# davidbau/rewriting

Measured on AMD Instinct MI355X. Metric: images/sec StyleGANv2-1024 fwd, higher is better.
Workload: dtype f32 (conv operands split into exact f16 pairs from 32x32 up, f32 accumulate); 1 GPU; stylegan2-1024 generator forward (FFHQ-1024 architecture); batch_per_gpu=64, mconv=seq, weights=synthetic seed 0, parallelism=seeds partitioned per rank, no collective, matrix_mode=split, direct_sums=auto

## Files before the change

include/rewriting_hip.h:

```cpp
#ifndef REWRITING_HIP_H
#define REWRITING_HIP_H

#include <stdint.h>

#ifdef __cplusplus
extern "C" {
#endif

typedef void* rw_stream_t;

#define RW_ERR_BAD_ARGUMENT 10001
#define RW_ERR_UNSUPPORTED  10002

int rw_abi_version(void);
const char* rw_error_string(int code);


int rw_fused_bias_act_f32(const float* x, const float* b, const float* ref, float* y,
                          int64_t n, int64_t step_b, int64_t size_b,
                          int act, int grad, float alpha, float scale, rw_stream_t stream);
int rw_fused_bias_act_f16(const uint16_t* x, const uint16_t* b, const uint16_t* ref, uint16_t* y,
                          int64_t n, int64_t step_b, int64_t size_b,
                          int act, int grad, float alpha, float scale, rw_stream_t stream);
int rw_fused_bias_act_f64(const double* x, const double* b, const double* ref, double* y,
// ... 120 lines not shown
int rw_conv_weight_wino4h_absmax_f32(const float* w, int out_ch, int in_ch, float* bound, rw_stream_t stream);
int rw_conv_transpose_blur_weight_wino4h_absmax_f32(const float* w, const float* k4, int out_ch, int in_ch, float* bound,
                                                    rw_stream_t stream);
int rw_conv_transpose_weight_winoh_absmax_f32(const float* w, int out_ch, int in_ch, float* bound, rw_stream_t stream);
int rw_dconv_weight_absmax_f32(const float* w, int out_ch, int in_ch, float* bound, rw_stream_t stream);
int rw_dconv_transpose_blur_weight_absmax_f32(const float* w, const float* k4, int out_ch, int in_ch, float* bound,
                                              rw_stream_t stream);
long long rw_packed_conv_weight_wino4h_elems(int out_ch, int in_ch);
int rw_pack_conv_weight_wino4h_f32(const float* w, float* uf, int out_ch, int in_ch, float u_scale, rw_stream_t stream);
int rw_conv3x3_wino4h_f32(const float* x, const float* uf, float* y, int batch, int in_ch, int out_ch, int h,
                          int w, float w_scale, const rw_conv_epilogue* ep, float u_inv, const float* x_amax,
                          float* y_amax, rw_stream_t stream);
int rw_conv3x3_wino4h_to_rgb_f32(const float* x, const float* uf, int batch, int in_ch, int out_ch, int h, int w,
                                 float w_scale, const rw_conv_epilogue* ep, const rw_rgb_epilogue* rgb, float u_inv,
                                 const float* x_amax, rw_stream_t stream);
long long rw_packed_conv_transpose_blur_wino4h_elems(int out_ch, int in_ch);
int rw_pack_conv_transpose_blur_weight_wino4h_f32(const float* w, const float* k4, float* uf, int out_ch, int in_ch,
                                                  float u_scale, rw_stream_t stream);
int rw_conv_transpose3x3s2_blur_wino4h_f32(const float* x, const float* uf, float* y, int batch, int in_ch,
                                           int out_ch, int h, int w, float w_scale, const rw_conv_epilogue* ep,
                                           const float* post_scale, float u_inv, const float* x_amax,
                                           float* y_amax, rw_stream_t stream);

int rw_dconv3x3_supported(int out_ch, int in_ch, int h, int w);
long long rw_packed_dconv_weight_elems(int out_ch, int in_ch);
int rw_pack_dconv_weight_f32(const float* w, float* wp, int out_ch, int in_ch, float u_scale, rw_stream_t stream);
int rw_dconv3x3_f32(const float* x, const float* wp, float* y, int batch, int in_ch, int out_ch, int h, int w,
                    float w_scale, const rw_conv_epilogue* ep, float u_inv, const float* x_amax, float* y_amax,
                    rw_stream_t stream);
int rw_dconv3x3_rgb_partials(int out_ch);
int rw_dconv3x3_rgb_partial_f32(const float* x, const float* wp, float* y, int batch, int in_ch, int out_ch, int h, int w,
                                float w_scale, const rw_conv_epilogue* ep, const rw_rgb_epilogue* rgb, float u_inv,
                                const float* x_amax, float* y_amax, rw_stream_t stream);
int rw_rgb_combine_f32(const float* partials, int n_part, const float* bias, const float* skip, float* y, int batch,
                       int64_t hw, rw_stream_t stream);
int rw_dconv3x3_to_rgb_supported(int out_ch, int in_ch, int h, int w);
int rw_dconv3x3_to_rgb_f32(const float* x, const float* wp, int batch, int in_ch, int out_ch, int h, int w,
                           float w_scale, const rw_conv_epilogue* ep, const rw_rgb_epilogue* rgb, float u_inv,
                           const float* x_amax, rw_stream_t stream);
int rw_dconv_transpose_blur_supported(int out_ch, int in_ch, int h, int w);
long long rw_packed_dconv_transpose_blur_weight_elems(int out_ch, int in_ch);
int rw_pack_dconv_transpose_blur_weight_f32(const float* w, const float* k4, float* wp, int out_ch, int in_ch,
                                            float u_scale, rw_stream_t stream);
int rw_dconv_transpose3x3s2_blur_f32(const float* x, const float* wp, float* y, int batch, int in_ch, int out_ch, int h,
                                     int w, float w_scale, const rw_conv_epilogue* ep, const float* post_scale,
                                     float u_inv, const float* x_amax, float* y_amax, rw_stream_t stream);

int rw_tconv_blur_supported(int out_ch, int in_ch, int h, int w);
int rw_tconv_blur_f32(const float* x, const float* wp, const float* k4, float* y, int batch, int in_ch, int out_ch, int h,
                      int w, float w_scale, const rw_conv_epilogue* ep, const float* post_scale, float u_inv,
// ... 154 lines not shown
```

rewriting_amd/_lib.py:

```python
import ctypes
import os
from ctypes import (POINTER, Structure, c_char_p, c_double, c_float, c_int, c_int32, c_int64, c_uint,
                    c_void_p)

_HERE = os.path.dirname(os.path.abspath(__file__))
LIB_PATH = os.environ.get('RW_HIP_LIB') or os.path.join(_HERE, 'librewriting_hip.so')

ABI_VERSION = 11


class ConvEpilogue(Structure):
    _fields_ = [('style', c_void_p), ('demod', c_void_p), ('noise', c_void_p),
                ('noise_w', c_void_p), ('bias', c_void_p), ('act', c_int)]


class RgbEpilogue(Structure):
    _fields_ = [('weight', c_void_p), ('style', c_void_p), ('bias', c_void_p), ('skip', c_void_p),
                ('out', c_void_p), ('scale', c_float)]


class SolveProblem(Structure):
    _fields_ = [
        ('out_ch', c_int), ('in_ch', c_int), ('h', c_int), ('w', c_int), ('rank', c_int),
        ('key', c_void_p), ('style', c_void_p), ('val', c_void_p), ('bias', c_void_p),
# ... 112 lines not shown
    'rw_pack_conv_transpose_blur_weight_wino4h_f32': (c_int, [c_void_p, c_void_p, c_void_p, c_int, c_int, c_float,
                                                              c_void_p]),
    'rw_conv_transpose3x3s2_blur_wino4h_f32': (c_int, [c_void_p, c_void_p, c_void_p, c_int, c_int, c_int, c_int,
                                                       c_int, c_float, POINTER(ConvEpilogue), c_void_p, c_float,
                                                       c_void_p, c_void_p, c_void_p]),
    'rw_dconv3x3_supported': (c_int, [c_int, c_int, c_int, c_int]),
    'rw_packed_dconv_weight_elems': (ctypes.c_longlong, [c_int, c_int]),
    'rw_pack_dconv_weight_f32': (c_int, [c_void_p, c_void_p, c_int, c_int, c_float, c_void_p]),
    'rw_dconv3x3_f32': (c_int, [c_void_p, c_void_p, c_void_p, c_int, c_int, c_int, c_int, c_int, c_float,
                                POINTER(ConvEpilogue), c_float, c_void_p, c_void_p, c_void_p]),
    'rw_dconv3x3_rgb_partials': (c_int, [c_int]),
    'rw_dconv3x3_rgb_partial_f32': (c_int, [c_void_p, c_void_p, c_void_p, c_int, c_int, c_int, c_int, c_int, c_float,
                                            POINTER(ConvEpilogue), POINTER(RgbEpilogue), c_float, c_void_p, c_void_p,
                                            c_void_p]),
    'rw_rgb_combine_f32': (c_int, [c_void_p, c_int, c_void_p, c_void_p, c_void_p, c_int, c_int64, c_void_p]),
    'rw_dconv3x3_to_rgb_supported': (c_int, [c_int, c_int, c_int, c_int]),
    'rw_dconv3x3_to_rgb_f32': (c_int, [c_void_p, c_void_p, c_int, c_int, c_int, c_int, c_int, c_float,
                                       POINTER(ConvEpilogue), POINTER(RgbEpilogue), c_float, c_void_p, c_void_p]),
    'rw_dconv_transpose_blur_supported': (c_int, [c_int, c_int, c_int, c_int]),
    'rw_packed_dconv_transpose_blur_weight_elems': (ctypes.c_longlong, [c_int, c_int]),
    'rw_pack_dconv_transpose_blur_weight_f32': (c_int, [c_void_p, c_void_p, c_void_p, c_int, c_int, c_float, c_void_p]),
    'rw_dconv_transpose3x3s2_blur_f32': (c_int, [c_void_p, c_void_p, c_void_p, c_int, c_int, c_int, c_int, c_int,
                                                 c_float, POINTER(ConvEpilogue), c_void_p, c_float, c_void_p, c_void_p,
                                                 c_void_p]),
    'rw_tconv_blur_supported': (c_int, [c_int, c_int, c_int, c_int]),
    'rw_tconv_blur_f32': (c_int, [c_void_p, c_void_p, c_void_p, c_void_p, c_int, c_int, c_int, c_int, c_int, c_float,
                                  POINTER(ConvEpilogue), c_void_p, c_float, c_void_p, c_void_p, c_void_p]),
    'rw_conv_transpose_blur_wino4_supported': (c_int, [c_int, c_int, c_int, c_int]),
    'rw_packed_conv_transpose_blur_wino4_elems': (ctypes.c_longlong, [c_int, c_int]),
    'rw_pack_conv_transpose_blur_weight_wino4_f32': (c_int, [c_void_p, c_void_p, c_void_p, c_int, c_int, c_void_p]),
# ... 79 lines not shown
```

rewriting_amd/csrc/rw_common.h:

```cpp
#pragma once
#include <hip/hip_runtime.h>
#include <stdint.h>
#include <stdlib.h>
#include "../../include/rewriting_hip.h"

#define RW_WAVE 64

#define RW_CHECK_ARG(cond) do { if (!(cond)) return RW_ERR_BAD_ARGUMENT; } while (0)
#define RW_LAUNCH_RESULT() ((int)hipGetLastError())

static inline hipStream_t rw_s(rw_stream_t s) { return (hipStream_t)s; }

static inline int64_t rw_cdiv(int64_t a, int64_t b) { return (a + b - 1) / b; }

static inline int rw_cu_count(void) {
  static int cached[64];
  int dev = 0;
  if (hipGetDevice(&dev) != hipSuccess || dev < 0 || dev >= 64) return 256;
  if (cached[dev] == 0) {
    int n = 0;
    cached[dev] = (hipDeviceGetAttribute(&n, hipDeviceAttributeMultiprocessorCount, dev) == hipSuccess && n > 0) ? n : 256;
  }
  return cached[dev];
}
// ... 197 lines not shown
__host__ __device__ __forceinline__ int rw_exp_above(float x) {
  const int e = (int)((__builtin_bit_cast(unsigned, x) >> 23) & 0xff) - 126;
  return e < -100 ? -100 : (e > 100 ? 100 : e);
}
template <int HEAD>
__host__ __device__ __forceinline__ void rw_split_scales(float am, float u_inv, float& in_scale, float& out_scale) {
  const int e = rw_exp_above(am);
  in_scale = __builtin_bit_cast(float, (unsigned)(127 + HEAD - e) << 23);
  out_scale = __builtin_bit_cast(float, (unsigned)(127 + e - HEAD) << 23) * u_inv;
}
static inline float rw_weight_scale_of(float u_absmax) {
  const int eu = u_absmax == 0.f ? 15 : rw_exp_above(u_absmax);
  return __builtin_bit_cast(float, (unsigned)(127 + 15 - eu) << 23);
}

static inline bool rw_epilogue_ok(const rw_conv_epilogue* ep) {
  return !ep || ((!ep->noise || ep->noise_w) && (!ep->act || ep->bias));
}
static inline bool rw_rgb_ok(const rw_rgb_epilogue* rgb) { return rgb && rgb->weight && rgb->style && rgb->out; }

template <class P> static inline void rw_fill_epilogue(P& p, const rw_conv_epilogue* ep) {
  p.style = ep ? ep->style : nullptr; p.demod = ep ? ep->demod : nullptr; p.noise = ep ? ep->noise : nullptr;
  p.noise_w = ep ? ep->noise_w : nullptr; p.bias = ep ? ep->bias : nullptr; p.act = ep ? ep->act : 0;
}
template <class P> static inline void rw_fill_rgb(P& p, const rw_rgb_epilogue* rgb) {
  p.rgb_weight = rgb ? rgb->weight : nullptr; p.rgb_style = rgb ? rgb->style : nullptr;
  p.rgb_bias = rgb ? rgb->bias : nullptr; p.rgb_skip = rgb ? rgb->skip : nullptr; p.rgb_out = rgb ? rgb->out : nullptr;
  p.rgb_scale = rgb ? rgb->scale : 0.f;
}

// ... 19 lines not shown
```

rewriting_amd/csrc/rw_ops.hip:

```cpp
#include "rw_common.h"
#ifndef OPS_NTS
#define OPS_NTS 0
#endif
#include <stdlib.h>
#include <stdint.h>

extern "C" int rw_abi_version(void) { return 11; }

extern "C" const char* rw_error_string(int code) {
  if (code == 0) return "success";
  if (code == RW_ERR_BAD_ARGUMENT) return "rewriting_hip: bad argument";
  if (code == RW_ERR_UNSUPPORTED) return "rewriting_hip: unsupported configuration";
  return hipGetErrorString((hipError_t)code);
}

template <typename T> struct RwAcc { typedef T type; };
template <> struct RwAcc<_Float16> { typedef float type; };

template <typename A>
__device__ __forceinline__ A rw_bias_act_one(A x, A ref, int code, A alpha, A scale) {
  A y;
  switch (code) {
    default:
    case 10: y = x; break;
// ... 1041 lines not shown
    }
    reinterpret_cast<float4*>(y)[q] = a;
  }
}

extern "C" int rw_rgb_combine_f32(const float* partials, int n_part, const float* bias, const float* skip, float* y,
                                  int batch, int64_t hw, rw_stream_t stream) {
  RW_CHECK_ARG(partials && y && n_part > 0 && batch > 0 && hw > 0);
  if (hw % 4) return RW_ERR_UNSUPPORTED;
  const int64_t n4 = (int64_t)batch * 3 * hw / 4;
  hipLaunchKernelGGL(rgb_combine_kernel, dim3(rw_stream_grid(n4, 256)), dim3(256), 0, rw_s(stream), partials, n_part, bias,
                     skip, y, n4, hw / 4, n4);
  return RW_LAUNCH_RESULT();
}

__global__ void __launch_bounds__(256) to_rgb_scalar_kernel(const float* __restrict__ x, const float* __restrict__ w,
                                                            const float* __restrict__ style,
                                                            const float* __restrict__ bias,
                                                            const float* __restrict__ skip, float* __restrict__ y,
                                                            int in_ch, int64_t hw, float w_scale) {
  extern __shared__ float wm[];
  const int b = blockIdx.y;
  for (int t = threadIdx.x; t < 3 * in_ch; t += 256) wm[t] = w_scale * w[t] * style[(int64_t)b * in_ch + t % in_ch];
  __syncthreads();
  const float* xb = x + (int64_t)b * in_ch * hw;
  for (int64_t q = (int64_t)blockIdx.x * 256 + threadIdx.x; q < hw; q += (int64_t)gridDim.x * 256) {
    float a[3] = {0.f, 0.f, 0.f};
    for (int i = 0; i < in_ch; ++i) {
      const float v = xb[(int64_t)i * hw + q];
      a[0] += wm[i] * v; a[1] += wm[in_ch + i] * v; a[2] += wm[2 * in_ch + i] * v;
// ... 31 lines not shown
```

rewriting_amd/csrc/rw_wino4.hip:

```cpp
#include "rw_common.h"

#ifndef W4_ABL
#define W4_ABL 0
#endif
#ifndef W4_SETPRIO
#define W4_SETPRIO 0
#endif

__host__ __device__ constexpr int w4_nat(int pos) { return pos < 18 ? pos : (pos < 26 ? pos + 10 : pos - 8); }

struct Wino4Problem {
  const float* x; const float* uf; float* y;
  const float* style; const float* demod; const float* noise; const float* noise_w; const float* bias;
  int batch, in_ch, out_ch, h, w;
  int groups_x, groups_y, gpw;
  float w_scale;
  int act;
  const float* rgb_weight; const float* rgb_style; const float* rgb_bias; const float* rgb_skip; float* rgb_out;
  float rgb_scale;
  const float* post;
  const float* x_amax; float* y_amax;
  float u_inv;
};

#define W4_PC 66
#define W4_RS 72

__device__ __forceinline__ void w4_bt(float& d0, float& d1, float& d2, float& d3, float& d4, float& d5) {
  const float t0 = 4.f * d0 - 5.f * d2 + d4;
  const float p = d4 - 4.f * d2, q = d3 - 4.f * d1;
  const float r = d4 - d2, s = 2.f * (d3 - d1);
  const float t5 = 4.f * d1 - 5.f * d3 + d5;
  d0 = t0; d1 = p + q; d2 = p - q; d3 = r + s; d4 = r - s; d5 = t5;
}

__device__ __forceinline__ void w4_bt2(rw_f32x2& d0, rw_f32x2& d1, rw_f32x2& d2, rw_f32x2& d3, rw_f32x2& d4,
                                       rw_f32x2& d5) {
// ... 822 lines not shown
    asm volatile("" ::: "memory");
    if (!mine) {
#pragma unroll
      for (int cc = 0; cc < 3; ++cc) *reinterpret_cast<rw_f32x4*>(&Ns[wave * NSZ + cc * 128 + slot]) = sum[cc];
    }
    __builtin_amdgcn_s_waitcnt(0xC07F);
    __builtin_amdgcn_s_barrier();
    asm volatile("" ::: "memory");
    if (mine) {
      const int64_t pix = (int64_t)(oy + lk) * p.w + ox;
#pragma unroll
      for (int cc = 0; cc < 3; ++cc) {
        const rw_f32x4 other = *reinterpret_cast<const rw_f32x4*>(&Ns[(wave ^ WGN) * NSZ + cc * 128 + slot]);
        const int64_t off = ((int64_t)ib * 3 + cc) * hw + pix;
        rw_f32x4 o4 = sum[cc] + other + (p.rgb_bias ? p.rgb_bias[cc] : 0.f);
        if (p.rgb_skip) o4 += *reinterpret_cast<const rw_f32x4*>(p.rgb_skip + off);
        *reinterpret_cast<rw_f32x4*>(p.rgb_out + off) = o4;
      }
    }
  };

  auto group_epilogue = [&](int g, int xs) __attribute__((always_inline)) {
    if (UP) { up_epilogue(g, xs); return; }
    if (RGB) { rgb_epilogue(g, xs); return; }
    const int oy = y0 + 4 * wn, ox = (gx0 + g) * 64 + 4 * lt;
    const float gain = p.act ? 1.4142135623730951f : 1.f, slope = p.act ? 0.2f : 1.f;
    rw_f32x4 nz[4];
#pragma unroll
    for (int r = 0; r < 4; ++r)
      nz[r] = p.noise ? *reinterpret_cast<const rw_f32x4*>(&Ns[wave * NSZ + 64 * r + 4 * lt]) * (noise_w * gain)
                      : rw_f32x4{0.f, 0.f, 0.f, 0.f};
// ... 451 lines not shown
}

extern "C" int rw_conv_transpose3x3s2_blur_wino4h_f32(const float* x, const float* uf, float* y, int batch, int in_ch,
                                                      int out_ch, int h, int w, float w_scale,
                                                      const rw_conv_epilogue* ep, const float* post_scale, float u_inv,
                                                      const float* x_amax, float* y_amax, rw_stream_t stream) {
  return up_wino4_launch(x, uf, y, batch, in_ch, out_ch, h, w, w_scale, ep, post_scale, true, u_inv, x_amax, y_amax, stream);
}

extern "C" int rw_conv3x3_wino4_to_rgb_supported(int out_ch, int in_ch, int h, int w) {
  return out_ch == 32 && in_ch <= 512 && wino4_shape_ok(out_ch, in_ch, h, w) ? 1 : 0;
}

static int wino4_to_rgb_launch(const float* x, const float* uf, int batch, int in_ch, int out_ch, int h, int w,
                               float w_scale, const rw_conv_epilogue* ep, const rw_rgb_epilogue* rgb, bool h16,
                               float u_inv, const float* x_amax, rw_stream_t stream) {
  RW_CHECK_ARG(x && uf && rw_rgb_ok(rgb) && batch > 0 && in_ch > 0 && out_ch > 0);
  RW_CHECK_ARG(rw_epilogue_ok(ep));
  RW_CHECK_ARG(!h16 || (x_amax && u_inv > 0.f));
  if (!rw_conv3x3_wino4_to_rgb_supported(out_ch, in_ch, h, w) || !w4_window_aligned(x)) return RW_ERR_UNSUPPORTED;
  Wino4Problem p = {};
  wino4_fill(p, x, uf, nullptr, batch, in_ch, out_ch, h, w, w_scale, ep, u_inv, x_amax, nullptr);
  rw_fill_rgb(p, rgb);
  p.gpw = wino4_gpw(p, batch, 1);
  const int64_t work = (int64_t)batch * p.groups_y * (p.groups_x / p.gpw);
  if (work <= 0 || work > 0x7fffffff) return RW_ERR_UNSUPPORTED;
  if (h16) {
    if (w4h_point_split(in_ch)) hipLaunchKernelGGL(conv_wino36h_rgb_ps_kernel, dim3((unsigned)work), dim3(256), 0, rw_s(stream), p);
    else hipLaunchKernelGGL(conv_wino36h_rgb_kernel, dim3((unsigned)work), dim3(256), 0, rw_s(stream), p);
    return RW_LAUNCH_RESULT();
  }
#if W4_PSPLIT
  if (w4_point_split()) {
    if (p.style) hipLaunchKernelGGL(conv_wino36_rgb_ps_kernel, dim3((unsigned)work), dim3(256), 0, rw_s(stream), p);
    else hipLaunchKernelGGL(conv_wino36_rgb_ns_ps_kernel, dim3((unsigned)work), dim3(256), 0, rw_s(stream), p);
  } else
#endif
  if (p.style) hipLaunchKernelGGL(conv_wino36_rgb_kernel, dim3((unsigned)work), dim3(256), 0, rw_s(stream), p);
  else hipLaunchKernelGGL(conv_wino36_rgb_ns_kernel, dim3((unsigned)work), dim3(256), 0, rw_s(stream), p);
  return RW_LAUNCH_RESULT();
}

extern "C" int rw_conv3x3_wino4_to_rgb_f32(const float* x, const float* uf, int batch, int in_ch, int out_ch, int h,
                                           int w, float w_scale, const rw_conv_epilogue* ep,
                                           const rw_rgb_epilogue* rgb, rw_stream_t stream) {
  return wino4_to_rgb_launch(x, uf, batch, in_ch, out_ch, h, w, w_scale, ep, rgb, false, 1.f, nullptr, stream);
}

extern "C" int rw_conv3x3_wino4h_to_rgb_f32(const float* x, const float* uf, int batch, int in_ch, int out_ch, int h,
                                            int w, float w_scale, const rw_conv_epilogue* ep,
                                            const rw_rgb_epilogue* rgb, float u_inv, const float* x_amax,
                                            rw_stream_t stream) {
  return wino4_to_rgb_launch(x, uf, batch, in_ch, out_ch, h, w, w_scale, ep, rgb, true, u_inv, x_amax, stream);
}
```

rewriting_amd/hip.py:

```python
import ctypes
from collections import namedtuple as _namedtuple

import torch

from . import _lib
from ._lib import ConvEpilogue, RgbEpilogue, SolveProblem, check

SQRT2 = 2 ** 0.5


def _stream():
    return ctypes.c_void_p(torch.cuda.current_stream().cuda_stream)


def _dev(t, name='tensor', dtype=torch.float32):
    if not isinstance(t, torch.Tensor):
        raise TypeError('%s must be a torch.Tensor' % name)
    if not t.is_cuda:
        raise RuntimeError('rewriting_amd: %s is on %s; the HIP kernels need a GPU tensor '
                           '(there is no CPU fallback)' % (name, t.device))
    if t.dtype != dtype:
        if dtype == torch.float32:
            raise RuntimeError('rewriting_amd: %s is %s; the C ABI is fp32 only (RW_ERR_UNSUPPORTED, include/rewriting_hip.h: '
                               'the reference\'s pybind modules also dispatch half and double, this library does not) -- '
# ... 235 lines not shown
def blur_noise_act(x, k4, noise, noise_w, bias, post_scale=None, y_amax=None):
    x = _dev(x, 'fmap')
    k4 = _dev(k4, 'blur kernel')
    noise = _opt(noise, 'noise')
    noise_w = _opt(noise_w, 'noise weight')
    bias = _opt(bias, 'bias')
    b, c, ih, iw = x.shape
    y = torch.empty(b, c, ih - 1, iw - 1, device=x.device, dtype=x.dtype)
    post_scale = _post_scale(post_scale, b, c, 'channels')
    y_amax = _amax_out(y_amax, y.numel())
    check(lib().rw_blur_noise_act_amax_f32(_p(x), _p(k4), _p(noise), _p(noise_w), _p(bias), _p(post_scale), _p(y),
                                           b, c, ih - 1, iw - 1, _p(y_amax), _stream()))
    return y


def rgb_combine(partials, bias, skip):
    partials = _dev(partials, 'rgb partial sums')
    bias = _opt(bias, 'rgb bias')
    skip = _opt(skip, 'rgb skip')
    n, b, c, h, w = partials.shape
    if c != 3 or (skip is not None and tuple(skip.shape) != (b, 3, h, w)):
        raise ValueError('rgb partial / skip shapes')
    y = torch.empty(b, 3, h, w, device=partials.device, dtype=partials.dtype)
    check(lib().rw_rgb_combine_f32(_p(partials), n, _p(bias), _p(skip), _p(y), b, h * w, _stream()))
    return y


BOUND_LANES = 64


def bound_floats(n_elems):
    return int(lib().rw_bound_floats(int(n_elems)))


def new_bound(n_elems, device):
    return torch.empty(bound_floats(n_elems), device=device, dtype=torch.float32)


# ... 200 lines not shown
    else:
        style_demod = [_opt(style_demod[0], 'style'), _opt(style_demod[1], 'demod')]
        args += [_p(t) for t in style_demod]
    if 'rgb' in slots:
        args.append(ctypes.byref(slots['rgb'][0]))
    if 'impl' in slots:
        args.append(int(slots['impl']))
    if 'post_scale' in slots:
        args.append(_p(slots['post_scale']))
    if u_inv is not None:
        x_amax = _amax_in(x, x_amax)
        args += [u_inv, _p(x_amax)]
        if 'y_amax' in slots:
            y_amax = _amax_out(slots['y_amax'], slots['y'].numel())
            args.append(_p(y_amax))
    entry = entries if isinstance(entries, str) else entries[u_inv is not None]
    check(getattr(lib(), entry)(*args, _stream()))


def _out(x, out_ch, up=1):
    b, _, h, w = x.shape
    return torch.empty(b, out_ch, up * h, up * w, device=x.device, dtype=x.dtype)


def _out_transposed(x, out_ch, out):
    b, _, h, w = x.shape
    y = out if out is not None else torch.empty(b, out_ch, 2 * h + 1, 2 * w + 1, device=x.device, dtype=x.dtype)
    if tuple(y.shape) != (b, out_ch, 2 * h + 1, 2 * w + 1) or not y.is_contiguous():
        raise ValueError('out has the wrong shape')
    return y
# ... 57 lines not shown
                  x_amax=None, y_amax=None):
    x = _dev(x, 'fmap')
    y = _out(x, out_ch)
    _conv(('rw_conv3x3_wino4_f32', 'rw_conv3x3_wino4h_f32'), x, _packed(uf, out_ch, x.shape[1], _WINO4), out_ch, w_scale,
          _epilogue(style, demod, noise, noise_w, bias, act), x_amax=x_amax, y=y, y_amax=y_amax)
    return y


wino4_to_rgb_supported = _supported('rw_conv3x3_wino4_to_rgb_supported', 'Shapes conv3x3_wino4_to_rgb takes: out_ch == 32')


def conv3x3_wino4_to_rgb(x, uf, out_ch, w_scale, rgb_weight, rgb_style, rgb_bias, rgb_skip, rgb_scale, style=None,
                         demod=None, noise=None, noise_w=None, bias=None, act=False, x_amax=None):
    x = _dev(x, 'fmap')
    rgb = _out(x, 3)
    _conv(('rw_conv3x3_wino4_to_rgb_f32', 'rw_conv3x3_wino4h_to_rgb_f32'), x, _packed(uf, out_ch, x.shape[1], _WINO4),
          out_ch, w_scale, _epilogue(style, demod, noise, noise_w, bias, act), x_amax=x_amax,
          rgb=_rgb_epilogue(rgb_weight, rgb_style, rgb_bias, rgb_skip, rgb_scale, rgb, x, out_ch))
    return None, rgb


def bf16x6_supported(out_ch, in_ch, width):
    return width >= 24 and in_ch % 16 == 0 and in_ch <= 1024 and out_ch % 64 == 0


def conv3x3_bf16x6(x, wb, out_ch, w_scale, style=None, demod=None, noise=None, noise_w=None, bias=None,
                   act=False):
    x = _dev(x, 'fmap')
    wb = _dev(wb, 'packed weight')
    if wb.numel() * 4 != lib().rw_packed_conv_weight_bf16x3_bytes(out_ch, x.shape[1]):
        raise ValueError('packed weight does not come from pack_conv_weight_bf16x3(%d x %d)' % (out_ch, x.shape[1]))
    y = _out(x, out_ch)
    _conv('rw_conv3x3_bf16x6_f32', x, (wb, None), out_ch, w_scale, _epilogue(style, demod, noise, noise_w, bias, act), y=y)
# ... 542 lines not shown
```

rewriting_amd/utils/stylegan2/models.py:

```python
import contextlib
import math
import re
import threading
import warnings
from collections import OrderedDict, namedtuple

import numpy as np
import torch
from torch import nn

from . import grad, op, routing
from .routing import switches
from ... import hip


_weight_epoch = [0]


def bump_weight_epoch():
    _weight_epoch[0] += 1


class _DerivedWeights:

# ... 85 lines not shown
                                  'tensors (the adjoints in utils/stylegan2/grad.py are float32); run it under '
                                  'torch.no_grad(), or differentiate a .float() model' % what)


def _unhooked(*modules):
    return all('forward' not in m.__dict__ for m in modules)


def _idle():
    return dict(
        stream=None,
        aux=None,
        keep=[],
        final=None,
        image_path=False,
        switches=None,
        neighbours={},
        pre={},
        pre_join=None)


class _RunningForward(threading.local):
    def __init__(self):
        vars(self).update(_idle())


_running = _RunningForward()
_side_streams = {}
_Neighbours = namedtuple('_Neighbours', 'reader successor torgb')
_NO_NEIGHBOURS = _Neighbours(None, None, None)
# ... 435 lines not shown


class UpsampleF(Upsample):
    def forward(self, d):
        return DataBag(d, fmap=super().forward(d.fmap))


class UpsampleO(Upsample):
    def __init__(self, kernel=[1, 3, 3, 1], factor=2):
        super().__init__(kernel, factor)

    def forward(self, d):
        side = _rgb_stream()
        if side is None:
            return DataBag(d, output=super().forward(d.output))
        with torch.cuda.stream(side):
            return DataBag(d, output=super().forward(d.output))


class NoiseInjectionF(nn.Module):
    def __init__(self):
        super().__init__()
        self.weight = nn.Parameter(torch.zeros(1))

    def noise_for(self, d, batch, height, width, device, double=False):
        noise = d.get('noise', None)
        if noise is None:
            rows = d.get('batch_rows', None)
            if rows is not None:
                start, total = rows
                return reference_noise(total, height * width, device, double)[start:start + batch]
            return reference_noise(batch, height * width, device, double)
# ... 82 lines not shown


class ToRGBF(nn.Module):

    def __init__(self, in_channel, style_dim, upsample=True, blur_kernel=[1, 3, 3, 1], skip=False):
        super().__init__()
        if upsample:
            self.upsample = Upsample(blur_kernel)
        self.conv = ModulatedConv2d(in_channel, 3, 1, style_dim, demodulate=False)
        self.bias = nn.Parameter(torch.zeros(1, 3, 1, 1))
        self.skip = skip

    def forward(self, d):
        if d.get('fused_rgb') is not None:
            return DataBag(d, output=d.fused_rgb, fused_rgb=None)
        if _double('ToRGBF', d.fmap, weight=self.conv.weight, bias=self.bias, style=d.style,
                   skip=d.get('output') if self.skip else None):
            return self._forward_f64(d)
        skip = d.output if self.skip else None
        if skip is not None and tuple(skip.shape[2:]) != tuple(d.fmap.shape[2:]):
            up = self.upsample if hasattr(self, 'upsample') else Upsample([1, 3, 3, 1]).to(skip.device)
            if _rgb_stream() is None:
                skip = up(skip)
            else:
                with torch.cuda.stream(_rgb_stream()):
                    skip = up(skip)
        conv = self.conv
        side = _rgb_stream()
        partials = d.get('rgb_partials')
        if partials is not None:
            if side is None:
                raise RuntimeError('ToRGB partial sums outside the forward that produces them')
            side.wait_stream(torch.cuda.current_stream())
            with torch.cuda.stream(side):
                out = hip.rgb_combine(partials, self.bias.view(3), skip)
# ... 153 lines not shown
        bound = dict(y_amax=y_amax) if y_amax is not None else {}
        if route.runs_layer:
            bound.update(dict(x_amax=x_amax) if route.split else {})
            out = dconv.run_whole_layer(fmap, style, route, fir, demod, noise=noise, post_scale=post, **bound,
                                        noise_w=self.noise.weight, bias=self.activate.bias, act=True)
        else:
            wide = dconv.run(fmap, style, style_on_load=True, demod=demod, x_amax=x_amax, route=route)
            out = hip.blur_noise_act(wide, fir, noise, self.noise.weight, self.activate.bias, post_scale=post, **bound)
        if y_amax is not None:
            out.rw_amax = (y_amax, out._version)
        return DataBag(d, style=style, fmap=out, **({} if post is None else dict(prescaled=post)))

    def _run_final(self, d, style, demod, x_amax, style_on_load, epilogue, route, received):
        _, torgb, idx = _running.final
        skip = d.output if torgb.skip else None
        if skip is not None and tuple(skip.shape[2:]) != tuple(d.fmap.shape[2:]):
            with _scope(final=None):
                return self.forward(received)
        main = torch.cuda.current_stream()
        if _running.stream is not None:
            main.wait_stream(_running.stream)
        rgb_style = _style_of(torgb, _prefetched(torgb), d.latent, idx)
        to_rgb = (torgb.conv.weight.view(3, torgb.conv.in_channel), rgb_style, torgb.bias.view(3), skip, torgb.conv.scale)
        _, rgb = self.mconv.dconv.run(d.fmap, style, style_on_load, demod=demod, x_amax=x_amax, to_rgb=to_rgb, route=route,
                                      **epilogue)
        return DataBag(d, style=style, fmap=None, fused_rgb=rgb)

    def _run_stride1(self, d, style, demod, ctx, x_amax, style_on_load, epilogue):
        fmap, (h, w) = d.fmap, d.fmap.shape[2:]
        route = self._route(ctx, h, w)
        y_amax = self._result_bound(ctx, fmap, h, w) if route.reports_bound else None
# ... 111 lines not shown
        mb, from_res = micro_batch()
        micro = (mb and fusion_enabled() and torch.is_tensor(input) and not self.bag_output
                 and not self.bag_input and input.shape[0] > mb and 'up_rgb%d' % (int(math.log2(from_res)) - 2)
                 in self._modules and _running.stream is None and _unhooked(*self.modules()))
        side_ok = (not micro and fusion_enabled() and _switches().rgb_stream and torch.is_tensor(input)
                   and input.is_cuda and not self.bag_output and _running.stream is None
                   and not torch.cuda.is_current_stream_capturing()
                   and _unhooked(*self.modules()))
        if not micro and not side_ok:
            return super().forward(input)
        final = (topology or self._topology())[1] if _switches().fuse_final_rgb else None
        if micro:
            return self._forward_micro(input, mb, from_res, final)
        with contextlib.ExitStack() as scopes:
            main = scopes.enter_context(_side_streams_joined(input.device))
            scopes.enter_context(_scope(final=final))
            out = input
            for name, module in self._modules.items():
                out = module(out)
                if name == 'latents' and _running.image_path and _switches().prefetch_styles:
                    scopes.enter_context(_scope(**self._prefetch_modulations(out, _running.aux)))
        if torch.is_tensor(out):
            out.record_stream(main)
        return out

    def _forward_micro(self, z, mb, from_res, final):
        mods = list(self._modules.values())
        k = list(self._modules).index('up_rgb%d' % (int(math.log2(from_res)) - 2))
        d = z
        for m in mods[:k]:
            d = m(d)
# ... 123 lines not shown
```

rewriting_amd/utils/stylegan2/routing.py:

```python
import os
from collections import namedtuple

from ... import hip

_CONV_IMPLS = {'auto': 0, 'mfma': 0, 'direct': 1, 'generic': 2, 'halo': 3, 'nosplitk': 5}
ONE_PASS_UP_MAX_IN = 64
FUSED_UP_MAX_IN = 512

Switches = namedtuple('Switches', [
    'fuse',
    'conv_impl',
    'conv_precision',
    'conv_algo',
    'up_algo',
    'mm',
    'mm_hooked_split',
    'mm_parts',
    'mm_direct16',
    'micro_batch',
    'up_fused',
    'up_fused2',
    'up_fused2_hooked',
    'up_fused2_max_in',
    'up_fused2_join',
    'direct16_small',
    'direct16_hooked',
    'dconv_ws_fwd',
    'dconv_v',
    'rgb_partial',
    'rgb_f4',
    'rgb_stream',
    'strip_stream',
    'side_priority',
    'prescale',
    'mm_no_handover',
    'prefetch_styles',
    'fuse_final_rgb',
])


def switches():
    env = os.environ.get
    direct16 = env('RW_MM_DIRECT16', 'auto')
    parts = env('RW_MM_PARTS')
    k, _, res = env('RW_MICRO_BATCH', '0').partition(':')
    return Switches(
        fuse=env('RW_FUSE', '1') != '0',
        conv_impl=_CONV_IMPLS[env('RW_CONV_IMPL', 'auto')],
        conv_precision=env('RW_CONV_PRECISION', 'f32'),
        conv_algo=env('RW_CONV_ALGO'),
        up_algo=env('RW_UP_ALGO', 'winograd'),
        mm=env('RW_MM'),
# ... 7 lines not shown
        up_fused2_max_in=int(env('RW_UP_FUSED2_MAX_IN', FUSED_UP_MAX_IN)),
        up_fused2_join=env('RW_UP_FUSED2_JOIN') == '1',
        direct16_small=env('RW_DIRECT16_SMALL', '1') != '0',
        direct16_hooked=env('RW_DIRECT16_HOOKED', '1') == '1',
        dconv_ws_fwd=env('RW_DCONV_WS_FWD', '1') != '0',
        dconv_v=env('RW_DCONV_V') == '1',
        rgb_partial=env('RW_RGB_PARTIAL', '1') != '0',
        rgb_f4=env('RW_RGB_F4', '1') != '0',
        rgb_stream=env('RW_RGB_STREAM', '1') != '0',
        strip_stream=env('RW_STRIP_STREAM', '1') != '0',
        side_priority=int(env('RW_SIDE_PRIORITY', '0')),
        prescale=env('RW_PRESCALE', '1') != '0',
        mm_no_handover=env('RW_MM_NO_HANDOVER') == '1',
        prefetch_styles=env('RW_PREFETCH_STYLES', '1') != '0',
        fuse_final_rgb=env('RW_FUSE_FINAL_RGB', '1') != '0',
    )


Context = namedtuple('Context', 'image_path on_device capturing rgb_stream aux_stream weight_changes')

STRIDE1_KERNELS = ('direct16', 'wino4_split', 'wino4', 'wino', 'bf16x6', 'gemm')
WHOLE_LAYER_KERNELS = ('fused', 'one_pass_direct16', 'one_pass_wino4')
UP_KERNELS = WHOLE_LAYER_KERNELS + ('f22_strips', 'halo_strips', 'plain')

Stride1Route = namedtuple('Stride1Route', 'kernel specialised rgb_partials reads_bound reports_bound prescaled')

UpRoute = namedtuple('UpRoute', 'kernel split side_strips reads_bound runs_layer')

FinalRgbRoute = namedtuple('FinalRgbRoute', 'kernel reads_bound')

# ... 112 lines not shown
```

Before: 1616 images/sec.

## Fuse RGB skip upsampling into ToRGB epilogue and partial combine

```diff
diff --git a/include/rewriting_hip.h b/include/rewriting_hip.h
--- a/include/rewriting_hip.h
+++ b/include/rewriting_hip.h
@@ -158,6 +158,12 @@
 int rw_conv3x3_wino4h_to_rgb_f32(const float* x, const float* uf, int batch, int in_ch, int out_ch, int h, int w,
                                  float w_scale, const rw_conv_epilogue* ep, const rw_rgb_epilogue* rgb, float u_inv,
                                  const float* x_amax, rw_stream_t stream);
+int rw_conv3x3_wino4_to_rgb_up_f32(const float* x, const float* uf, int batch, int in_ch, int out_ch, int h, int w,
+                                   float w_scale, const rw_conv_epilogue* ep, const rw_rgb_epilogue* rgb,
+                                   const float* skip_half, const float* k4, rw_stream_t stream);
+int rw_conv3x3_wino4h_to_rgb_up_f32(const float* x, const float* uf, int batch, int in_ch, int out_ch, int h, int w,
+                                    float w_scale, const rw_conv_epilogue* ep, const rw_rgb_epilogue* rgb, float u_inv,
+                                    const float* x_amax, const float* skip_half, const float* k4, rw_stream_t stream);
 long long rw_packed_conv_transpose_blur_wino4h_elems(int out_ch, int in_ch);
 int rw_pack_conv_transpose_blur_weight_wino4h_f32(const float* w, const float* k4, float* uf, int out_ch, int in_ch,
                                                   float u_scale, rw_stream_t stream);
@@ -178,6 +184,8 @@
                                 const float* x_amax, float* y_amax, rw_stream_t stream);
 int rw_rgb_combine_f32(const float* partials, int n_part, const float* bias, const float* skip, float* y, int batch,
                        int64_t hw, rw_stream_t stream);
+int rw_rgb_combine_up_f32(const float* partials, int n_part, const float* bias, const float* skip_half, const float* k4,
+                          float* y, int batch, int h, int w, rw_stream_t stream);
 int rw_dconv3x3_to_rgb_supported(int out_ch, int in_ch, int h, int w);
 int rw_dconv3x3_to_rgb_f32(const float* x, const float* wp, int batch, int in_ch, int out_ch, int h, int w,
                            float w_scale, const rw_conv_epilogue* ep, const rw_rgb_epilogue* rgb, float u_inv,
diff --git a/rewriting_amd/_lib.py b/rewriting_amd/_lib.py
--- a/rewriting_amd/_lib.py
+++ b/rewriting_amd/_lib.py
@@ -150,6 +150,14 @@
                                             POINTER(ConvEpilogue), POINTER(RgbEpilogue), c_float, c_void_p, c_void_p,
                                             c_void_p]),
     'rw_rgb_combine_f32': (c_int, [c_void_p, c_int, c_void_p, c_void_p, c_void_p, c_int, c_int64, c_void_p]),
+    'rw_rgb_combine_up_f32': (c_int, [c_void_p, c_int, c_void_p, c_void_p, c_void_p, c_void_p, c_int, c_int, c_int,
+                                      c_void_p]),
+    'rw_conv3x3_wino4_to_rgb_up_f32': (c_int, [c_void_p, c_void_p, c_int, c_int, c_int, c_int, c_int, c_float,
+                                               POINTER(ConvEpilogue), POINTER(RgbEpilogue), c_void_p, c_void_p,
+                                               c_void_p]),
+    'rw_conv3x3_wino4h_to_rgb_up_f32': (c_int, [c_void_p, c_void_p, c_int, c_int, c_int, c_int, c_int, c_float,
+                                                POINTER(ConvEpilogue), POINTER(RgbEpilogue), c_float, c_void_p, c_void_p,
+                                                c_void_p, c_void_p]),
     'rw_dconv3x3_to_rgb_supported': (c_int, [c_int, c_int, c_int, c_int]),
     'rw_dconv3x3_to_rgb_f32': (c_int, [c_void_p, c_void_p, c_int, c_int, c_int, c_int, c_int, c_float,
                                        POINTER(ConvEpilogue), POINTER(RgbEpilogue), c_float, c_void_p, c_void_p]),
diff --git a/rewriting_amd/csrc/rw_common.h b/rewriting_amd/csrc/rw_common.h
--- a/rewriting_amd/csrc/rw_common.h
+++ b/rewriting_amd/csrc/rw_common.h
@@ -235,6 +235,36 @@
   return __builtin_bit_cast(float, (unsigned)(127 + 15 - eu) << 23);
 }
 
+__device__ __forceinline__ void rw_up2k4_row4(const float* __restrict__ xm, int hh, int hw, int oy, int ox,
+                                              const float* __restrict__ kf, float (&acc)[4]) {
+  acc[0] = acc[1] = acc[2] = acc[3] = 0.f;
+  const int m = ox >> 1;
+  const bool okl = m >= 1, okr = m + 2 < hw;
+#pragma unroll
+  for (int j = 0; j < 2; ++j) {
+    const int vy = oy + (oy & 1) + 2 * j - 2, iy = vy >> 1;
+    const bool row = vy >= 0 && iy < hh;
+    const float* xr = xm + (int64_t)(row ? iy : 0) * hw + m;
+    const float* kr = kf + 4 * (3 - (oy & 1) - 2 * j);
+    const float k0 = kr[3], k1 = kr[2], k2 = kr[1], k3 = kr[0];
+    const float xl = xr[okl ? -1 : 0], x0 = xr[0], x1 = xr[1], x2 = xr[okr ? 2 : 1];
+    float t[4] = {acc[0], acc[1], acc[2], acc[3]};
+    t[0] += xl * k0;
+    t[0] = okl ? t[0] : acc[0];
+    t[0] += x0 * k2;
+    t[1] += x0 * k1;
+    t[1] += x1 * k3;
+    t[2] += x0 * k0;
+    t[2] += x1 * k2;
+    t[3] += x1 * k1;
+    float u = t[3];
+    u += x2 * k3;
+    t[3] = okr ? u : t[3];
+#pragma unroll
+    for (int e = 0; e < 4; ++e) acc[e] = row ? t[e] : acc[e];
+  }
+}
+
 static inline bool rw_epilogue_ok(const rw_conv_epilogue* ep) {
   return !ep || ((!ep->noise || ep->noise_w) && (!ep->act || ep->bias));
 }
diff --git a/rewriting_amd/csrc/rw_ops.hip b/rewriting_amd/csrc/rw_ops.hip
--- a/rewriting_amd/csrc/rw_ops.hip
+++ b/rewriting_amd/csrc/rw_ops.hip
@@ -1079,6 +1079,41 @@
   return RW_LAUNCH_RESULT();
 }
 
+__global__ void __launch_bounds__(256) rgb_combine_up_kernel(const float* __restrict__ part, int n_part,
+                                                             const float* __restrict__ bias,
+                                                             const float* __restrict__ half,
+                                                             const float* __restrict__ k4, float* __restrict__ y,
+                                                             int64_t n4, int h, int w, int64_t stride4) {
+  const int w4 = w >> 2, hh = h >> 1, hw = w >> 1;
+  for (int64_t q = (int64_t)blockIdx.x * 256 + threadIdx.x; q < n4; q += (int64_t)gridDim.x * 256) {
+    float4 a = reinterpret_cast<const float4*>(part)[q];
+    for (int j = 1; j < n_part; ++j) {
+      const float4 v = reinterpret_cast<const float4*>(part)[q + j * stride4];
+      a.x += v.x; a.y += v.y; a.z += v.z; a.w += v.w;
+    }
+    const int64_t row = q / w4;
+    const int64_t plane = row / h;
+    if (bias) {
+      const float bv = bias[plane % 3];
+      a.x += bv; a.y += bv; a.z += bv; a.w += bv;
+    }
+    float up[4];
+    rw_up2k4_row4(half + plane * hh * hw, hh, hw, (int)(row - plane * h), (int)(q - row * w4) * 4, k4, up);
+    a.x += up[0]; a.y += up[1]; a.z += up[2]; a.w += up[3];
+    reinterpret_cast<float4*>(y)[q] = a;
+  }
+}
+
+extern "C" int rw_rgb_combine_up_f32(const float* partials, int n_part, const float* bias, const float* skip_half,
+                                     const float* k4, float* y, int batch, int h, int w, rw_stream_t stream) {
+  RW_CHECK_ARG(partials && skip_half && k4 && y && n_part > 0 && batch > 0 && h > 0 && w > 0);
+  if (w % 4 || h % 2) return RW_ERR_UNSUPPORTED;
+  const int64_t n4 = (int64_t)batch * 3 * h * w / 4;
+  hipLaunchKernelGGL(rgb_combine_up_kernel, dim3(rw_stream_grid(n4, 256)), dim3(256), 0, rw_s(stream), partials, n_part,
+                     bias, skip_half, k4, y, n4, h, w, n4);
+  return RW_LAUNCH_RESULT();
+}
+
 __global__ void __launch_bounds__(256) to_rgb_scalar_kernel(const float* __restrict__ x, const float* __restrict__ w,
                                                             const float* __restrict__ style,
                                                             const float* __restrict__ bias,
diff --git a/rewriting_amd/csrc/rw_wino4.hip b/rewriting_amd/csrc/rw_wino4.hip
--- a/rewriting_amd/csrc/rw_wino4.hip
+++ b/rewriting_amd/csrc/rw_wino4.hip
@@ -21,6 +21,7 @@
   const float* post;
   const float* x_amax; float* y_amax;
   float u_inv;
+  const float* rgb_fir;
 };
 
 #define W4_PC 66
@@ -873,7 +874,16 @@
         const rw_f32x4 other = *reinterpret_cast<const rw_f32x4*>(&Ns[(wave ^ WGN) * NSZ + cc * 128 + slot]);
         const int64_t off = ((int64_t)ib * 3 + cc) * hw + pix;
         rw_f32x4 o4 = sum[cc] + other + (p.rgb_bias ? p.rgb_bias[cc] : 0.f);
-        if (p.rgb_skip) o4 += *reinterpret_cast<const rw_f32x4*>(p.rgb_skip + off);
+        if (p.rgb_fir) {
+          float up[4];
+          int uy = oy + lk, ux = ox, ub = ib, uh = p.h, uw = p.w;
+          asm volatile("" : "+v"(uy), "+v"(ux), "+s"(ub), "+s"(uh), "+s"(uw));
+          rw_up2k4_row4(p.rgb_skip + ((int64_t)ub * 3 + cc) * ((int64_t)(uh >> 1) * (uw >> 1)), uh >> 1, uw >> 1, uy, ux,
+                        p.rgb_fir, up);
+          o4 += rw_f32x4{up[0], up[1], up[2], up[3]};
+        } else if (p.rgb_skip) {
+          o4 += *reinterpret_cast<const rw_f32x4*>(p.rgb_skip + off);
+        }
         *reinterpret_cast<rw_f32x4*>(p.rgb_out + off) = o4;
       }
     }
@@ -1355,14 +1365,17 @@
 
 static int wino4_to_rgb_launch(const float* x, const float* uf, int batch, int in_ch, int out_ch, int h, int w,
                                float w_scale, const rw_conv_epilogue* ep, const rw_rgb_epilogue* rgb, bool h16,
-                               float u_inv, const float* x_amax, rw_stream_t stream) {
+                               float u_inv, const float* x_amax, const float* skip_half, const float* k4,
+                               rw_stream_t stream) {
   RW_CHECK_ARG(x && uf && rw_rgb_ok(rgb) && batch > 0 && in_ch > 0 && out_ch > 0);
+  RW_CHECK_ARG(!skip_half || (k4 && !rgb->skip));
   RW_CHECK_ARG(rw_epilogue_ok(ep));
   RW_CHECK_ARG(!h16 || (x_amax && u_inv > 0.f));
   if (!rw_conv3x3_wino4_to_rgb_supported(out_ch, in_ch, h, w) || !w4_window_aligned(x)) return RW_ERR_UNSUPPORTED;
   Wino4Problem p = {};
   wino4_fill(p, x, uf, nullptr, batch, in_ch, out_ch, h, w, w_scale, ep, u_inv, x_amax, nullptr);
   rw_fill_rgb(p, rgb);
+  if (skip_half) { p.rgb_skip = skip_half; p.rgb_fir = k4; }
   p.gpw = wino4_gpw(p, batch, 1);
   const int64_t work = (int64_t)batch * p.groups_y * (p.groups_x / p.gpw);
   if (work <= 0 || work > 0x7fffffff) return RW_ERR_UNSUPPORTED;
@@ -1385,12 +1398,32 @@
 extern "C" int rw_conv3x3_wino4_to_rgb_f32(const float* x, const float* uf, int batch, int in_ch, int out_ch, int h,
                                            int w, float w_scale, const rw_conv_epilogue* ep,
                                            const rw_rgb_epilogue* rgb, rw_stream_t stream) {
-  return wino4_to_rgb_launch(x, uf, batch, in_ch, out_ch, h, w, w_scale, ep, rgb, false, 1.f, nullptr, stream);
+  return wino4_to_rgb_launch(x, uf, batch, in_ch, out_ch, h, w, w_scale, ep, rgb, false, 1.f, nullptr, nullptr, nullptr,
+                             stream);
 }
 
 extern "C" int rw_conv3x3_wino4h_to_rgb_f32(const float* x, const float* uf, int batch, int in_ch, int out_ch, int h,
                                             int w, float w_scale, const rw_conv_epilogue* ep,
                                             const rw_rgb_epilogue* rgb, float u_inv, const float* x_amax,
                                             rw_stream_t stream) {
-  return wino4_to_rgb_launch(x, uf, batch, in_ch, out_ch, h, w, w_scale, ep, rgb, true, u_inv, x_amax, stream);
-}
+  return wino4_to_rgb_launch(x, uf, batch, in_ch, out_ch, h, w, w_scale, ep, rgb, true, u_inv, x_amax, nullptr, nullptr,
+                             stream);
+}
+
+extern "C" int rw_conv3x3_wino4_to_rgb_up_f32(const float* x, const float* uf, int batch, int in_ch, int out_ch, int h,
+                                              int w, float w_scale, const rw_conv_epilogue* ep,
+                                              const rw_rgb_epilogue* rgb, const float* skip_half, const float* k4,
+                                              rw_stream_t stream) {
+  RW_CHECK_ARG(skip_half && k4);
+  return wino4_to_rgb_launch(x, uf, batch, in_ch, out_ch, h, w, w_scale, ep, rgb, false, 1.f, nullptr, skip_half, k4,
+                             stream);
+}
+
+extern "C" int rw_conv3x3_wino4h_to_rgb_up_f32(const float* x, const float* uf, int batch, int in_ch, int out_ch, int h,
+                                               int w, float w_scale, const rw_conv_epilogue* ep,
+                                               const rw_rgb_epilogue* rgb, float u_inv, const float* x_amax,
+                                               const float* skip_half, const float* k4, rw_stream_t stream) {
+  RW_CHECK_ARG(skip_half && k4);
+  return wino4_to_rgb_launch(x, uf, batch, in_ch, out_ch, h, w, w_scale, ep, rgb, true, u_inv, x_amax, skip_half, k4,
+                             stream);
+}
diff --git a/rewriting_amd/hip.py b/rewriting_amd/hip.py
--- a/rewriting_amd/hip.py
+++ b/rewriting_amd/hip.py
@@ -273,14 +273,31 @@
     return y
 
 
+HalfSkip = _namedtuple('HalfSkip', 'image fir')
+
+
+def _half_skip(skip, b, h, w):
+    image, fir = _dev(skip.image, 'rgb skip (half size)'), _dev(skip.fir, 'upsampling kernel')
+    if tuple(image.shape) != (b, 3, h // 2, w // 2) or h % 2 or w % 2 or tuple(fir.shape) != (4, 4):
+        raise ValueError('half-size rgb skip / kernel shapes')
+    return HalfSkip(image, fir)
+
+
 def rgb_combine(partials, bias, skip):
     partials = _dev(partials, 'rgb partial sums')
     bias = _opt(bias, 'rgb bias')
+    n, b, c, h, w = partials.shape
+    y = torch.empty(b, 3, h, w, device=partials.device, dtype=partials.dtype)
+    if isinstance(skip, HalfSkip):
+        if c != 3:
+            raise ValueError('rgb partial / skip shapes')
+        skip = _half_skip(skip, b, h, w)
+        check(lib().rw_rgb_combine_up_f32(_p(partials), n, _p(bias), _p(skip.image), _p(skip.fir), _p(y), b, h, w,
+                                          _stream()))
+        return y
     skip = _opt(skip, 'rgb skip')
-    n, b, c, h, w = partials.shape
     if c != 3 or (skip is not None and tuple(skip.shape) != (b, 3, h, w)):
         raise ValueError('rgb partial / skip shapes')
-    y = torch.empty(b, 3, h, w, device=partials.device, dtype=partials.dtype)
     check(lib().rw_rgb_combine_f32(_p(partials), n, _p(bias), _p(skip), _p(y), b, h * w, _stream()))
     return y
 
@@ -511,6 +528,8 @@
         if 'y_amax' in slots:
             y_amax = _amax_out(slots['y_amax'], slots['y'].numel())
             args.append(_p(y_amax))
+    if 'half_skip' in slots:
+        args += [_p(slots['half_skip'].image), _p(slots['half_skip'].fir)]
     entry = entries if isinstance(entries, str) else entries[u_inv is not None]
     check(getattr(lib(), entry)(*args, _stream()))
 
@@ -598,9 +617,13 @@
                          demod=None, noise=None, noise_w=None, bias=None, act=False, x_amax=None):
     x = _dev(x, 'fmap')
     rgb = _out(x, 3)
-    _conv(('rw_conv3x3_wino4_to_rgb_f32', 'rw_conv3x3_wino4h_to_rgb_f32'), x, _packed(uf, out_ch, x.shape[1], _WINO4),
+    entries, up = ('rw_conv3x3_wino4_to_rgb_f32', 'rw_conv3x3_wino4h_to_rgb_f32'), {}
+    if isinstance(rgb_skip, HalfSkip):
+        entries = ('rw_conv3x3_wino4_to_rgb_up_f32', 'rw_conv3x3_wino4h_to_rgb_up_f32')
+        up, rgb_skip = dict(half_skip=_half_skip(rgb_skip, x.shape[0], x.shape[2], x.shape[3])), None
+    _conv(entries, x, _packed(uf, out_ch, x.shape[1], _WINO4),
           out_ch, w_scale, _epilogue(style, demod, noise, noise_w, bias, act), x_amax=x_amax,
-          rgb=_rgb_epilogue(rgb_weight, rgb_style, rgb_bias, rgb_skip, rgb_scale, rgb, x, out_ch))
+          rgb=_rgb_epilogue(rgb_weight, rgb_style, rgb_bias, rgb_skip, rgb_scale, rgb, x, out_ch), **up)
     return None, rgb
 
 
diff --git a/rewriting_amd/utils/stylegan2/models.py b/rewriting_amd/utils/stylegan2/models.py
--- a/rewriting_amd/utils/stylegan2/models.py
+++ b/rewriting_amd/utils/stylegan2/models.py
@@ -123,6 +123,7 @@
         keep=[],
         final=None,
         image_path=False,
+        inline_up=False,
         switches=None,
         neighbours={},
         pre={},
@@ -588,8 +589,18 @@
         side = _rgb_stream()
         if side is None:
             return DataBag(d, output=super().forward(d.output))
+        if (_running.inline_up and d.output.dtype is torch.float32 and self.factor == 2
+                and tuple(self.kernel.shape) == (4, 4)):
+            return DataBag(d, output=hip.HalfSkip(d.output, self.kernel))
         with torch.cuda.stream(side):
             return DataBag(d, output=super().forward(d.output))
+
+
+def _full_size(skip):
+    if not isinstance(skip, hip.HalfSkip):
+        return skip
+    with torch.cuda.stream(_rgb_stream()):
+        return op.upfirdn2d(skip.image, skip.fir, up=2, down=1, pad=(2, 1))
 
 
 class NoiseInjectionF(nn.Module):
@@ -702,11 +713,13 @@
     def forward(self, d):
         if d.get('fused_rgb') is not None:
             return DataBag(d, output=d.fused_rgb, fused_rgb=None)
+        skip = d.get('output') if self.skip else None
+        if isinstance(skip, hip.HalfSkip) and d.get('rgb_partials') is None:
+            skip = _full_size(skip)
         if _double('ToRGBF', d.fmap, weight=self.conv.weight, bias=self.bias, style=d.style,
-                   skip=d.get('output') if self.skip else None):
+                   skip=skip.image if isinstance(skip, hip.HalfSkip) else skip):
             return self._forward_f64(d)
-        skip = d.output if self.skip else None
-        if skip is not None and tuple(skip.shape[2:]) != tuple(d.fmap.shape[2:]):
+        if torch.is_tensor(skip) and tuple(skip.shape[2:]) != tuple(d.fmap.shape[2:]):
             up = self.upsample if hasattr(self, 'upsample') else Upsample([1, 3, 3, 1]).to(skip.device)
             if _rgb_stream() is None:
                 skip = up(skip)
@@ -890,7 +903,9 @@
     def _run_final(self, d, style, demod, x_amax, style_on_load, epilogue, route, received):
         _, torgb, idx = _running.final
         skip = d.output if torgb.skip else None
-        if skip is not None and tuple(skip.shape[2:]) != tuple(d.fmap.shape[2:]):
+        if isinstance(skip, hip.HalfSkip) and route.kernel not in ('wino4', 'wino4_split'):
+            skip = _full_size(skip)
+        if torch.is_tensor(skip) and tuple(skip.shape[2:]) != tuple(d.fmap.shape[2:]):
             with _scope(final=None):
                 return self.forward(received)
         main = torch.cuda.current_stream()
@@ -1032,7 +1047,9 @@
             return self._forward_micro(input, mb, from_res, final)
         with contextlib.ExitStack() as scopes:
             main = scopes.enter_context(_side_streams_joined(input.device))
-            scopes.enter_context(_scope(final=final))
+            inline_up = (_running.image_path and _switches().rgb_inline_up
+                         and not any(m._forward_hooks or m._forward_pre_hooks for m in self.modules()))
+            scopes.enter_context(_scope(final=final, inline_up=inline_up))
             out = input
             for name, module in self._modules.items():
                 out = module(out)
diff --git a/rewriting_amd/utils/stylegan2/routing.py b/rewriting_amd/utils/stylegan2/routing.py
--- a/rewriting_amd/utils/stylegan2/routing.py
+++ b/rewriting_amd/utils/stylegan2/routing.py
@@ -36,6 +36,7 @@
     'mm_no_handover',
     'prefetch_styles',
     'fuse_final_rgb',
+    'rgb_inline_up',
 ])
 
 
@@ -73,6 +74,7 @@
         mm_no_handover=env('RW_MM_NO_HANDOVER') == '1',
         prefetch_styles=env('RW_PREFETCH_STYLES', '1') != '0',
         fuse_final_rgb=env('RW_FUSE_FINAL_RGB', '1') != '0',
+        rgb_inline_up=env('RW_RGB_INLINE_UP', '1') != '0',
     )
 
 
```

After: 1642 images/sec (median of 6 runs). 1.6% higher.
